# lim0606/pytorch-ardae-vae

Hardware: AMD Instinct MI355X
Metric: AR-DAE-VAE train-steps/sec (batch 512, nz_cdae 256) on dbMNIST (higher is better)
Workload: dtype f32; 1 GPU; BASELINE config #2: MNISTIPVAE mlp z=32 h=256 + cDAE mlp-grad h=256 L=3, global batch 512, nz_cdae 256 (131072 rows), dynamic binarisation on device, 1 cDAE + 1 VAE update per step; global_batch=512, nz_cdae=256, per_gpu_batch=512, parallelism=dp1

## Files before the change

### include/ardae_hip.h

```cpp
#ifndef ARDAE_HIP_H
#define ARDAE_HIP_H

#include <stddef.h>
#include <stdint.h>

#ifdef __cplusplus
extern "C" {
#endif

#define ARDAE_ABI_VERSION 1

enum { ARDAE_ACT_NONE = 0, ARDAE_ACT_RELU = 1, ARDAE_ACT_SOFTPLUS = 2, ARDAE_ACT_ELU = 3, ARDAE_ACT_TANH = 4, ARDAE_ACT_LEAKY_RELU = 5, ARDAE_ACT_SWISH = 6 };

enum {
  ARDAE_EPI_ACT = 0,
  ARDAE_EPI_DACT = 1,
  ARDAE_EPI_CHAIN = 2,
  ARDAE_EPI_DAE_LOSS = 3
};

typedef struct ardae_lin_src {
  const float* x;
  int ld;
  int K;
// ... 157 lines not shown
  int act;
  int flags;
} ardae_model_desc;
enum { ARDAE_MODEL_NO_CENTER = 1,
       ARDAE_MODEL_HEAD_SHIFT = 1, ARDAE_MODEL_HEAD_MASK = 7 << 1,
       ARDAE_MODEL_CLIPPED = 16,
       ARDAE_MODEL_CLIP_Z0_SHIFT = 8, ARDAE_MODEL_CLIP_Z_SHIFT = 12, ARDAE_MODEL_CLIP_MASK = 0xff00 };
size_t ardae_model_param_floats(const ardae_model_desc* d);
size_t ardae_model_packed_floats(const ardae_model_desc* d);
size_t ardae_model_workspace_floats(const ardae_model_desc* d, int B, int nz, int mode);
int ardae_model_pack(const ardae_model_desc* d, const float* params, float* packed, void* stream);
int ardae_model_encode(const ardae_model_desc* d, const float* params, const float* packed, const float* x,
                       const float* noise, int B, int nz, float* workspace, size_t workspace_floats, float* z_out,
                       void* stream);
int ardae_model_encode_pair(const ardae_model_desc* d, const float* params, const float* packed, const float* x,
                            const float* noise, int B, int nz, float* workspace, size_t workspace_floats, float* z0_out,
                            float* z_out, int phase, void* stream);
int ardae_model_vae_forward(const ardae_model_desc* d, const float* params, const float* packed, const float* x,
                            const float* noise, int B, int nz, float beta, float* workspace, size_t workspace_floats,
                            float* z_out, float* losses, void* stream);
int ardae_model_vae_forward_dev(const ardae_model_desc* d, const float* params, const float* packed, const float* x,
                                const float* noise, int B, int nz, const void* state, float* workspace, size_t workspace_floats,
                                float* z_out, float* losses, void* stream);
int ardae_model_encode_hidden(const ardae_model_desc* d, const float* params, const float* packed, const float* x, int B,
                              float* workspace, size_t workspace_floats, float* z0_out, float* hidden_out, void* stream);
int ardae_model_encode_hidden_raw(const ardae_model_desc* d, const float* params, const float* packed, const float* x, const float* raw0, int B,
                                  float* workspace, size_t workspace_floats, float* z0_out, float* hidden_out, void* stream);
int ardae_model_decode(const ardae_model_desc* d, const float* params, const float* packed, const float* z, int R,
                       float* workspace, size_t workspace_floats, float* out0, float* out1, void* stream);
int ardae_model_loss_rows(const ardae_model_desc* d, const float* out0, const float* out1, const float* x, const float* z,
                          int rows, int nz, float* recon_row, float* prior_row, void* stream);
int ardae_model_vae_backward(const ardae_model_desc* d, const float* params, const float* packed, const float* x,
                             const float* noise, int B, int nz, float beta, float dloss, const float* dz_extra,
                             float* workspace, size_t workspace_floats, float* grads, float grads_beta, void* stream);
int ardae_model_vae_backward_dev(const ardae_model_desc* d, const float* params, const float* packed, const float* x,
                                 const float* noise, int B, int nz, const void* state, float dloss, const float* dz_extra,
                                 float* workspace, size_t workspace_floats, float* grads, float grads_beta, void* stream);
int ardae_model_vae_backward_decoder(const ardae_model_desc* d, const float* params, const float* packed, const float* x,
                                     const float* noise, int B, int nz, float beta, float dloss, float* workspace,
                                     size_t workspace_floats, void* stream);
int ardae_model_vae_backward_sampler(const ardae_model_desc* d, const float* params, const float* packed, const float* x,
                                     const float* noise, int B, int nz, const float* dz_extra, float seed_scale,
                                     float* workspace, size_t workspace_floats, float* grads, float grads_beta, void* stream);
int ardae_model_vae_backward_decoder_dev(const ardae_model_desc* d, const float* params, const float* packed, const float* x,
                                         const float* noise, int B, int nz, const void* state, float dloss, float* workspace,
                                         size_t workspace_floats, void* stream);
// ... 93 lines not shown
```

### pytorch-ardae-vae_amd/csrc/host_util.h

```cpp
#pragma once
#include <algorithm>
#include <cstring>
#include <vector>

#include "common.h"
#include "elementwise.h"
#include "linear.h"
#include "wgrad.h"

namespace ardae {

inline size_t al64(size_t n) { return (n + 63) & ~size_t(63); }
inline unsigned nblk(int64_t n) { return (unsigned)((n + 255) / 256); }

struct Bump {
  float* base; size_t cap; size_t off = 0; bool ok = true;
  Bump(float* b, size_t c) : base(b), cap(c) {}
  Bump() : base(nullptr), cap(~size_t(0) >> 2) {}
  float* take(size_t n) {
    size_t o = off; off += al64(n);
    if (off > cap) { ok = false; return base; }
    return base ? base + o : nullptr;
  }
};

inline int lin1(int epi, int act, int M, int Nout, const float* x, int ldx, int K, const float* wp, LinArgs a, hipStream_t st) {
  a.M = M; a.Nout = Nout; a.nsrc = 1; a.act = act;
  a.src[0].x = x; a.src[0].ld = ldx; a.src[0].K = K; a.src[0].wp = wp;
  return launch_linear(a, epi, st);
}
inline int lin2(int epi, int act, int M, int Nout, const float* x0, int ld0, int K0, const float* wp0, const float* x1, int ld1, int K1, const float* wp1,
                LinArgs a, hipStream_t st) {
  a.M = M; a.Nout = Nout; a.nsrc = 2; a.act = act;
  a.src[0].x = x0; a.src[0].ld = ld0; a.src[0].K = K0; a.src[0].wp = wp0;
  a.src[1].x = x1; a.src[1].ld = ld1; a.src[1].K = K1; a.src[1].wp = wp1;
  return launch_linear(a, epi, st);
}

inline int dense_fwd(int act, int M, int n, const float* x, int ldx, int K, const float* wp, const float* bias, float* y, hipStream_t st) {
  LinArgs A{}; A.bias = bias; A.Y = y; A.ldY = n;
  return lin1(EPI_ACT, act, M, n, x, ldx, K, wp, A, st);
}
inline int dense_bwd(int act, int M, int n, const float* g, int K, const float* wp, const float* S, float* y, hipStream_t st, const float* Q = nullptr) {
  LinArgs A{}; A.S = S; A.ldS = n; A.Q = Q; A.ldQ = Q ? n : 0; A.Y = y; A.ldY = n;
  return lin1(EPI_DACT, act, M, n, g, K, K, wp, A, st);
}
inline int dense_bwd2(int act, int M, int n, const float* g0, const float* wp0, const float* g1, const float* wp1, int K, const float* S, float* y,
                      hipStream_t st) {
  LinArgs A{}; A.S = S; A.ldS = n; A.Y = y; A.ldY = n;
  return lin2(EPI_DACT, act, M, n, g0, K, K, wp0, g1, K, K, wp1, A, st);
}

struct Lin { size_t w, b; int out, in; };
inline Lin next_lin(size_t& off, int out, int in, int nbias = -1) {
  Lin l; l.out = out; l.in = in; l.w = off; off += (size_t)out * in; l.b = off; off += nbias < 0 ? out : nbias;
  return l;
}

struct PackList {
  std::vector<PackItem> items;
  const float* params; float* packed;
  size_t off = 0;
  PackList() : params(nullptr), packed(nullptr) {}
  PackList(const float* params_, float* packed_) : params(params_), packed(packed_) {}
// ... 82 lines not shown
       CAP_HIDDEN_RAW = 4 };
struct Family {
  int (*desc_check)(const ardae_model_desc* d);
  unsigned (*caps)(const ardae_model_desc& d);
  size_t (*param_floats)(const ardae_model_desc&);
  size_t (*packed_floats)(const ardae_model_desc&);
  size_t (*workspace_floats)(const ardae_model_desc&, int B, int nz, int mode);
  int (*pack)(const ardae_model_desc&, const float* params, float* packed, hipStream_t);
  int (*encode)(const ardae_model_desc&, const float* params, const float* packed, const float* x, const float* noise, int B, int nz,
                float* workspace, size_t wsf, float* z_out, float* hidden_out, hipStream_t, const float* raw0);
  int (*decode)(const ardae_model_desc&, const float* params, const float* packed, const float* z, int R, float* workspace, size_t wsf,
                float* out0, hipStream_t, float* out1);
  int (*vae_forward)(const ardae_model_desc&, const float* params, const float* packed, const float* x, const float* noise, int B, int nz,
                     DevFloat beta, float* workspace, size_t wsf, float* z_out, float* losses, hipStream_t);
  int (*vae_backward)(const ardae_model_desc&, const float* params, const float* packed, const float* x, const float* noise, int B, int nz,
                      DevFloat beta, float dloss, const float* dz_extra, float* workspace, size_t wsf, float* grads, float grads_beta, hipStream_t);
  const GaussFamily* gauss;
  int (*encode_pair)(const ardae_model_desc&, const float* params, const float* packed, const float* x, const float* noise, int B, int nz,
                     float* workspace, size_t wsf, float* z0_out, float* z_out, int phase, hipStream_t);
  int (*vae_backward_decoder)(const ardae_model_desc&, const float* params, const float* packed, const float* x, const float* noise, int B, int nz,
                              DevFloat beta, float dloss, float* workspace, size_t wsf, hipStream_t);
  int (*vae_backward_sampler)(const ardae_model_desc&, const float* params, const float* packed, const float* x, const float* noise, int B, int nz,
                              const float* dz_extra, DevFloat seed_scale, float* workspace, size_t wsf, float* grads, float grads_beta, hipStream_t);
};
inline unsigned no_caps(const ardae_model_desc&) { return 0; }
inline int desc_flags_ok(const ardae_model_desc* d, int allowed) {
  ARDAE_CHECK_ARG((d->flags & ~allowed) == 0,
                  "model: unknown flags %d (ARDAE_MODEL_NO_CENTER / the sampler-head bits / ARDAE_MODEL_CLIPPED: residual-conv kinds 5 / 6 only; "
                  "the log-variance clip codes: kinds 3 / 7 only)", d->flags);
  ARDAE_CHECK_ARG(((d->flags >> ARDAE_MODEL_CLIP_Z0_SHIFT) & 15) <= 10 && ((d->flags >> ARDAE_MODEL_CLIP_Z_SHIFT) & 15) <= 10, "model: unknown log-variance clip code");
  return 0;
}
const Family* family_of(int kind);
inline const Family& family(const ardae_model_desc* d) { return *family_of(d->kind); }

template <class Layout, class Packed> size_t family_param_floats(const ardae_model_desc& d) { return Layout(d).total; }
template <class Layout, class Packed> size_t family_packed_floats(const ardae_model_desc& d) {
  const Layout P(d);
  PackList pl;
  const Packed K(P, pl);
  return pl.total();
}
template <class Layout, class Packed> int family_pack(const ardae_model_desc& d, const float* params, float* packed, hipStream_t st) {
  const Layout P(d);
  PackList pl(params, packed);
  const Packed K(P, pl);
// ... 15 lines not shown
```

### pytorch-ardae-vae_amd/csrc/ipmodel.h

```cpp
#pragma once
#include "host_util.h"
#include "mlp.h"

namespace ardae {

struct IpBufs { float *z, *out0, *out1, *dout0, *dout1, *dzq, *dz, *rec_row, *pri_row; };

struct IpEncodeOut { float* z_out; float* hidden_out; const float* raw0; bool std0; };

struct IpTraitsBase {
  static constexpr bool mlp_decoder = false;
  static constexpr bool direct_z = false;
  struct Grads { float* grads; float beta; };
  template <class Entry> static Grads grads_of(Entry&, const float*, const float*, float* grads, float grads_beta) { return {grads, grads_beta}; }
  template <class Layout> static size_t extra_floats(const Layout&, int, int, int) { return 0; }
  template <class Layout> static int rows_ok(const Layout&, int, bool) { return 0; }
  template <class Entry> static int hidden_copy(Entry&, float*, int, hipStream_t) { return 0; }
};

template <class F> size_t ip_workspace_floats(const ardae_model_desc& d, int B, int nz, int mode) {
  const typename F::Layout P(d);
  const typename F::Packed K(P);
  if constexpr (F::mlp_decoder)
    if (mode == 2) return K.dec.decode_floats((size_t)B * nz);
  const int m = mode == 3 ? 0 : mode;
  Bump ws;
  typename F::Ws W{};
  carve(P, K, ws, B, nz, m, W);
  if (m == 1) {
    WgradList wl(nullptr);
    F::wgrads(P, K, W, nullptr, nullptr, B, nz, wl, ws);
  }
  return ws.off + F::extra_floats(P, B, nz, mode);
}

template <class F> int ip_encode(const ardae_model_desc& d, const float* params, const float* packed, const float* x, const float* noise, int B, int nz,
                                 float* workspace, size_t wsf, float* z_out, float* hidden_out, hipStream_t st, const float* raw0) {
  typename F::Entry entry(d, workspace, wsf, B, nz, 0);
  auto& [P, K, ws, W] = entry;
  const size_t nn = F::noise_floats(P, B, nz);
  float* zero = noise ? nullptr : F::zero_noise(entry, nn);
  ARDAE_CHECK_ARG(ws.ok, "model_encode: internal workspace accounting error");
  ARDAE_TRY(F::rows_ok(P, nz, true));
  ARDAE_CHECK_ARG(!hidden_out || nz == 1, "model_encode: the hidden context is defined for nz == 1");
  const IpEncodeOut enc{z_out, hidden_out, raw0, noise == nullptr};
  ARDAE_TRY(noise_or_zero(noise, zero, nn, st));
  ARDAE_TRY(F::sampler_fwd(entry, params, packed, x, noise, B, nz, &enc, st));
  if (z_out && !F::direct_z) ARDAE_TRY(launch_copy(F::bufs(W).z, (size_t)B * nz * d.z_dim, z_out, st));
  if (hidden_out) ARDAE_TRY(F::hidden_copy(entry, hidden_out, B, st));
  return 0;
}

template <class F> int ip_decode(const ardae_model_desc& d, const float* params, const float* packed, const float* z, int R, float* workspace, size_t wsf,
                                 float* out0, hipStream_t st, float*) {
  typename F::Entry entry(d, workspace, wsf, R, 1, 2);
  ARDAE_CHECK_ARG(entry.ws.ok, "model_decode: internal workspace accounting error");
  ARDAE_TRY(F::decoder_fwd(entry, params, packed, z, R, st));
  return launch_copy(F::bufs(entry.W).out0, (size_t)R * d.input_dim, out0, st);
}

template <class F> int ip_vae_forward(const ardae_model_desc& d, const float* params, const float* packed, const float* x, const float* noise, int B, int nz,
                                      DevFloat beta, float* workspace, size_t wsf, float* z_out, float* losses, hipStream_t st) {
  typename F::Entry entry(d, workspace, wsf, B, nz, 1);
  auto& [P, K, ws, W] = entry;
  ARDAE_CHECK_ARG(ws.ok, "model_vae_forward: internal workspace accounting error");
  ARDAE_TRY(F::rows_ok(P, nz, false));
  const IpBufs G = F::bufs(W);
  const int R = B * nz;
  ARDAE_TRY(F::sampler_fwd(entry, params, packed, x, noise, B, nz, nullptr, st));
  ARDAE_TRY(launch_copy(G.z, (size_t)R * d.z_dim, z_out, st));
  ARDAE_TRY(F::decoder_fwd(entry, params, packed, G.z, R, st));
  ARDAE_TRY(launch_vae_loss(G.out1 ? 1 : 0, G.out0, G.out1, x, G.z, R, nz, d.input_dim, d.z_dim, beta, 0, 0.f, nullptr, G.rec_row, G.pri_row, nullptr,
                            nullptr, nullptr, st));
  return launch_vae_loss_finalize(G.rec_row, G.pri_row, R, beta, losses, st);
}

template <class F> int ip_backward(const ardae_model_desc& d, const float* params, const float* packed, const float* x, const float* noise, int B, int nz,
                                   DevFloat beta, float dloss, const float* dz_extra, DevFloat seed_scale, float* workspace, size_t wsf, float* grads,
                                   float grads_beta, int phases, hipStream_t st) {
  typename F::Entry entry(d, workspace, wsf, B, nz, 1);
  ARDAE_CHECK_ARG(entry.ws.ok, "model_vae_backward: internal workspace accounting error");
  typename F::Grads g = F::grads_of(entry, params, packed, grads, grads_beta);
  const IpBufs G = F::bufs(entry.W);
  const int R = B * nz;
  if (phases & 1) {
    ARDAE_TRY(launch_vae_loss(G.out1 ? 1 : 0, G.out0, G.out1, x, G.z, R, nz, d.input_dim, d.z_dim, beta, 1, dloss / (float)R,
                              phases == 3 ? dz_extra : nullptr, G.rec_row, G.pri_row, G.dout0, G.dout1, G.dzq, st));
    ARDAE_TRY(F::decoder_bwd(entry, packed, R, g, st));
  }
  if (!(phases & 2)) return 0;
  if (phases == 2 && dz_extra) ARDAE_TRY(launch_axpy(dz_extra, (int64_t)R * d.z_dim, seed_scale, G.dz, st));
  return F::sampler_bwd(entry, params, packed, x, noise, B, nz, g, st);
}
template <class F> int ip_vae_backward(const ardae_model_desc& d, const float* params, const float* packed, const float* x, const float* noise, int B,
                                       int nz, DevFloat beta, float dloss, const float* dz_extra, float* workspace, size_t wsf, float* grads,
                                       float grads_beta, hipStream_t st) {
  return ip_backward<F>(d, params, packed, x, noise, B, nz, beta, dloss, dz_extra, 1.f, workspace, wsf, grads, grads_beta, 3, st);
// ... 25 lines not shown
```

### pytorch-ardae-vae_amd/csrc/mlp.h

```cpp
#pragma once
#include <vector>

#include "host_util.h"

namespace ardae {

struct MlpStack {
  std::vector<Lin> lin;
  std::vector<size_t> f, b;
  MlpStack() {}
  MlpStack(const Lin* l, size_t n, PackList& pl) : lin(l, l + n), f(n), b(n) {
    for (size_t i = 0; i < n; ++i) pl.pair(lin[i], f[i], b[i]);
  }
  size_t n() const { return lin.size(); }

  int fwd(const float* params, const float* packed, int act, int M, const float* x, float* const* a, hipStream_t st, size_t first = 1) const {
    for (size_t l = first; l <= n(); ++l) {
      const Lin& L = lin[l - 1];
      ARDAE_TRY(dense_fwd(act, M, L.out, l == 1 ? x : a[l - 1], L.in, L.in, packed + f[l - 1], params + L.b, a[l], st));
    }
    return 0;
  }
  int bwd(const float* packed, int act, int M, float* const* a, float* const* d, hipStream_t st) const {
    for (size_t l = n(); l >= 2; --l) ARDAE_TRY(dense_bwd(act, M, lin[l - 1].in, d[l], lin[l - 1].out, packed + b[l - 1], a[l - 1], d[l - 1], st));
    return 0;
  }
  void wgrads(WgradList& wl, int M, const float* x, float* const* a, float* const* d) const {
    for (size_t l = 1; l <= n(); ++l) {
      const Lin& L = lin[l - 1];
      wl.push(M, L.out, L.in, d[l], l == 1 ? x : a[l - 1], L.in, wl.g(L.w), L.in, wl.g(L.b));
    }
  }
  void carve(Bump& ws, size_t M, std::vector<float*>& a) const {
    a.assign(n() + 1, nullptr);
    for (size_t l = 1; l <= n(); ++l) a[l] = ws.take(M * lin[l - 1].out);
  }
};

struct MlpDecoder {
  MlpStack stack;
  Lin head[2];
  size_t head_f[2], head_b[2];
  int nh = 0;
// ... 73 lines not shown
```

### pytorch-ardae-vae_amd/csrc/model.hip

```cpp
#include <vector>

#include "ardae_hip.h"
#include "common.h"
#include "auxconvvae.h"
#include "auxmodel.h"
#include "auxvae.h"
#include "convmodel.h"
#include "convvae.h"
#include "resmodel.h"
#include "vaemodel.h"
#include "ipmodel.h"
#include "elementwise.h"
#include "mlp.h"

namespace ardae {
namespace {

struct ModelLayout {
  int kind, D, nd, h, zd, nl, act;
  std::vector<Lin> inp, stack, dec, heads;
  std::vector<bool> stack_noise;
  size_t total = 0;
  explicit ModelLayout(const ardae_model_desc& d)
      : kind(d.kind), D(d.input_dim), nd(d.noise_dim), h(d.h_dim), zd(d.z_dim), nl(d.n_layers), act(d.act) {
// ... 43 lines not shown
  float *rec_row, *pri_row;
  std::vector<float*> dt, de;
  float* drb;
};

void carve(const ModelLayout& P, const ModelPacked& K, Bump& ws, int B, int nz, int mode, ModelWs& W) {
  const size_t R = (size_t)B * nz, h = P.h;
  W.x2 = ws.take((size_t)B * P.D);
  K.inp.carve(ws, B, W.e);
  W.rb = ws.take((size_t)B * h);
  W.t.assign(P.stack.size(), nullptr);
  for (size_t i = 1; i < P.stack.size(); ++i) W.t[i] = ws.take(R * h);
  W.z = ws.take(R * P.zd);
  if (mode == 0) return;
  K.dec.carve(ws, R, true, W.D);
  W.rec_row = ws.take(R); W.pri_row = ws.take(R);
  W.dt.assign(P.stack.size(), nullptr);
  for (size_t i = 1; i < P.stack.size(); ++i) W.dt[i] = ws.take(R * h);
  K.inp.carve(ws, B, W.de);
  W.drb = ws.take((size_t)B * h);
}
using MlpEntry = Entry<ModelLayout, ModelPacked, ModelWs>;

int encode_trunk(const ModelLayout& P, const ModelPacked& K, const float* params, const float* packed, const float* x, int B,
                 ModelWs& W, hipStream_t st) {
  const int h = P.h;
  const float* x_in = x;
  if (P.kind == 0) {
    ARDAE_TRY(launch_affine(x, (int64_t)B * P.D, 2.f, -1.f, W.x2, st));
    x_in = W.x2;
  }
  ARDAE_TRY(K.inp.fwd(params, packed, P.act, B, x_in, W.e.data(), st));
  return dense_fwd(ACT_NONE, B, h, W.e[P.inp.size()], h, h, packed + K.sh_f[0], params + P.stack[0].b, W.rb, st);
}

int encode_stack(const ModelLayout& P, const ModelPacked& K, const float* params, const float* packed, const float* noise,
                 int B, int nz, const float* rb, const std::vector<float*>& t, float* zdst, bool keep_hidden, hipStream_t st) {
  const int R = B * nz, h = P.h, act = P.act;
  const size_t ns = P.stack.size();
  if (!keep_hidden && ns == 2 && P.stack_noise[0] && !P.stack_noise[1] && P.stack[0].out == h) {
    LinArgs A{}; A.M = R; A.Nout = h; A.act = act; A.nsrc = 1;
    A.rowbias = rb; A.rowbias_ld = h; A.rows_per_group = nz;
    A.src[0].x = noise; A.src[0].ld = P.nd; A.src[0].K = P.nd; A.src[0].wp = packed + K.sn_f[0];
    if (sampler_tail_eligible(A, P.stack[1].out))
      return launch_sampler_tail(A, packed + K.sh_f[1], params + P.stack[1].b, zdst, P.stack[1].out, P.stack[1].out, st);
  }
  for (size_t i = 0; i < ns; ++i) {
    const bool last = i + 1 == ns;
    const int out = P.stack[i].out;
    LinArgs A{}; A.Y = last ? zdst : t[i + 1]; A.ldY = out; A.M = R; A.Nout = out; A.act = last ? ACT_NONE : act;
    int n = 0;
    if (i == 0) {
      A.rowbias = rb; A.rowbias_ld = h; A.rows_per_group = nz;
    } else {
      A.bias = params + P.stack[i].b;
      A.src[n].x = t[i]; A.src[n].ld = h; A.src[n].K = h; A.src[n].wp = packed + K.sh_f[i]; ++n;
// ... 10 lines not shown
struct MlpTraits : IpTraitsBase {
  using Layout = ModelLayout; using Packed = ModelPacked; using Ws = ModelWs; using Entry = MlpEntry;
  static constexpr bool mlp_decoder = true;
  static constexpr bool direct_z = true;
  static int desc_check(const ardae_model_desc* d) { return mlp_desc_check(d, 0); }
  static unsigned caps(const ardae_model_desc& d) { return d.kind == 1 ? CAP_GAUSS_DECODER : 0; }
  static IpBufs bufs(const ModelWs& W) { return {W.z, W.D.o[0], W.D.o[1], W.D.dox[0], W.D.dox[1], W.D.dzq, W.D.dz, W.rec_row, W.pri_row}; }
  static void wgrads(const ModelLayout& P, const ModelPacked& K, const ModelWs& W, const float* x, const float* noise, int B, int nz, WgradList& wl, Bump& ws) {
    const int R = B * nz, h = P.h;
    const size_t ns = P.stack.size();
    K.dec.wgrads(wl, R, W.z, W.D);
    for (size_t i = 0; i < ns; ++i) {
      const Lin& L = P.stack[i];
      const float* G = (i == ns - 1) ? W.D.dz : W.dt[i + 1];
      if (i == 0) wl.push(B, L.out, h, W.drb, W.e[P.inp.size()], h, wl.g(L.w), L.in, nullptr);
      else wl.push(R, L.out, h, G, W.t[i], h, wl.g(L.w), L.in, P.stack_noise[i] ? nullptr : wl.g(L.b));
      if (P.stack_noise[i]) wl.push(R, L.out, P.nd, G, noise, P.nd, wl.g(L.w + h), L.in, wl.g(L.b));
    }
    K.inp.wgrads(wl, B, P.kind == 0 ? W.x2 : x, W.e.data(), W.de.data());
    wl.assign(ws, (int)(P.heads.size() + P.dec.size() + 2 * ns + P.inp.size()));
  }
  static size_t extra_floats(const ModelLayout& P, int B, int nz, int mode) {
    if (mode == 3) return (P.stack.size() - 1) * al64((size_t)B * P.h) + al64((size_t)B * P.nd);
    return al64((size_t)B * nz * P.nd);
  }
  static size_t noise_floats(const ModelLayout& P, int B, int nz) { return (size_t)B * nz * P.nd; }
  static float* zero_noise(Entry& e, size_t n) { return e.ws.take(n); }
  static int sampler_fwd(Entry& e, const float* params, const float* packed, const float* x, const float* noise, int B, int nz, const IpEncodeOut* enc,
                         hipStream_t st) {
    ARDAE_TRY(encode_trunk(e.P, e.K, params, packed, x, B, e.W, st));
    return encode_stack(e.P, e.K, params, packed, noise, B, nz, e.W.rb, e.W.t, enc && enc->z_out ? enc->z_out : e.W.z, enc == nullptr, st);
  }
  static int decoder_fwd(Entry& e, const float* params, const float* packed, const float* z, int R, hipStream_t st) {
    return e.K.dec.fwd(params, packed, e.P.act, R, z, e.W.D.hid.data(), e.W.D.o, st);
  }
  static int decoder_bwd(Entry& e, const float* packed, int R, Grads&, hipStream_t st) { return e.K.dec.bwd(packed, e.P.act, R, e.W.D, st); }
  static int sampler_bwd(Entry& e, const float*, const float* packed, const float* x, const float* noise, int B, int nz, Grads& g, hipStream_t st) {
    auto& [P, K, ws, W] = e;
    const int R = B * nz, h = P.h, act = P.act;
    const size_t ns = P.stack.size(), ninp = P.inp.size();
    for (size_t i = ns - 1; i >= 1; --i)
      ARDAE_TRY(dense_bwd(act, R, h, (i == ns - 1) ? W.D.dz : W.dt[i + 1], P.stack[i].out, packed + K.sh_b[i], W.t[i], W.dt[i], st));
    ARDAE_TRY(launch_segment_sum(W.dt[1], h, B, nz, h, 1.0f, W.drb, h, st));
    ARDAE_TRY(dense_bwd(act, B, h, W.drb, h, packed + K.sh_b[0], W.e[ninp], W.de[ninp], st));
    ARDAE_TRY(K.inp.bwd(packed, act, B, W.e.data(), W.de.data(), st));
    WgradList wl(g.grads, g.beta);
    wgrads(P, K, W, x, noise, B, nz, wl, ws);
    ARDAE_CHECK_ARG(ws.ok, "model_vae_backward: internal workspace accounting error");
    return wl.launch(st);
  }
};

int mlp_encode_pair(const ardae_model_desc& d, const float* params, const float* packed, const float* x, const float* noise, int B, int nz,
                    float* workspace, size_t wsf, float* z0_out, float* z_out, int phase, hipStream_t st) {
  MlpEntry entry(d, workspace, wsf, B, nz, 0);
  auto& [P, K, ws, W] = entry;
  std::vector<float*> t0(P.stack.size(), nullptr);
  for (size_t i = 1; i < P.stack.size(); ++i) t0[i] = ws.take((size_t)B * P.h);
  float* zero = ws.take((size_t)B * P.nd);
  ARDAE_CHECK_ARG(ws.ok, "model_encode_pair: internal workspace accounting error");
  if (phase != 2) {
    ARDAE_TRY(launch_fill(zero, (size_t)B * P.nd, 0.f, st));
    ARDAE_TRY(encode_trunk(P, K, params, packed, x, B, W, st));
    ARDAE_TRY(encode_stack(P, K, params, packed, zero, B, 1, W.rb, t0, z0_out, false, st));
  }
  if (phase != 1) ARDAE_TRY(encode_stack(P, K, params, packed, noise, B, nz, W.rb, W.t, z_out, false, st));
  return 0;
}

constexpr Family mlp_family() {
  Family f = ip_family<MlpTraits>();
  f.encode_pair = mlp_encode_pair;
  f.vae_backward_decoder = ip_vae_backward_decoder<MlpTraits>;
  f.vae_backward_sampler = ip_vae_backward_sampler<MlpTraits>;
  return f;
}
const Family MLP_FAMILY = mlp_family();

}

const Family* family_of(int kind) {
  static const Family* const by_kind[20] = {&MLP_FAMILY, &MLP_FAMILY, &CONV_FAMILY, &AUX_FAMILY, &AUXCONV_FAMILY, &RES_FAMILY, &RES_FAMILY, &AUX_FAMILY,
                                            &VAE_FAMILY, &VAE_FAMILY, nullptr, &CONVVAE_FAMILY, &RESVAE_FAMILY, nullptr, &AUXVAE_FAMILY,
                                            &AUXVAE_FAMILY, nullptr, &AUXCONVVAE_FAMILY, nullptr, &AUXRESVAE_FAMILY};
  return kind >= 0 && kind <= 19 ? by_kind[kind] : nullptr;
}

}

using namespace ardae;

static int desc_ok(const ardae_model_desc* d) {
  ARDAE_CHECK_ARG(d != nullptr, "model: desc is NULL");
  ARDAE_CHECK_ARG(family_of(d->kind) != nullptr,
                  "model: kind must be 0 (MNISTIPVAE), 1 (ToyIPVAE concat), 2 (ConvIPVAE), 3 (MNISTAuxIPVAE), 4 (MNISTConvAuxIPVAE), 5 (ResConvIPVAE), "
// ... 66 lines not shown
int ardae_model_decode(const ardae_model_desc* d, const float* params, const float* packed, const float* z, int R, float* workspace,
                       size_t workspace_floats_, float* out0, float* out1, void* stream) {
  ARDAE_TRY(desc_ok(d));
  ARDAE_CHECK_ARG(params && packed && z && workspace && out0 && R > 0, "model_decode: bad arguments");
  ARDAE_CHECK_ARG(!(family(d).caps(*d) & CAP_GAUSS_DECODER) || out1, "model_decode: the Gaussian decoder needs out1 (logvar)");
  ARDAE_CHECK_ARG(workspace_floats_ >= family(d).workspace_floats(*d, R, 1, 2), "model_decode: workspace too small");
  return family(d).decode(*d, params, packed, z, R, workspace, workspace_floats_, out0, (hipStream_t)stream, out1);
}

int ardae_model_loss_rows(const ardae_model_desc* d, const float* out0, const float* out1, const float* x, const float* z, int rows,
                          int nz, float* recon_row, float* prior_row, void* stream) {
  ARDAE_TRY(desc_ok(d));
  return launch_vae_loss(family(d).caps(*d) & CAP_GAUSS_DECODER ? 1 : 0, out0, out1, x, z, rows, nz, d->input_dim, d->z_dim, 1.f, 0, 0.f, nullptr, recon_row, prior_row, nullptr,
                         nullptr, nullptr, (hipStream_t)stream);
}

static int vae_forward_entry(const ardae_model_desc* d, const float* params, const float* packed, const float* x, const float* noise, int B,
                             int nz, DevFloat beta, float* workspace, size_t workspace_floats_, float* z_out, float* losses, void* stream) {
  ARDAE_TRY(model_common(d, params, packed, x, B, nz, workspace, workspace_floats_, 1));
  ARDAE_CHECK_ARG(noise && z_out && losses, "model_vae_forward: null pointer argument");
  return family(d).vae_forward(*d, params, packed, x, noise, B, nz, beta, workspace, workspace_floats_, z_out, losses, (hipStream_t)stream);
}

static int vae_backward_entry(const ardae_model_desc* d, const float* params, const float* packed, const float* x, const float* noise, int B,
                              int nz, DevFloat beta, float dloss, const float* dz_extra, float* workspace, size_t workspace_floats_,
                              float* grads, float grads_beta, void* stream) {
  ARDAE_TRY(model_common(d, params, packed, x, B, nz, workspace, workspace_floats_, 1));
  ARDAE_CHECK_ARG(noise && grads, "model_vae_backward: null pointer argument");
  return family(d).vae_backward(*d, params, packed, x, noise, B, nz, beta, dloss, dz_extra, workspace, workspace_floats_, grads, grads_beta,
                                (hipStream_t)stream);
}

static int vae_backward_decoder_entry(const ardae_model_desc* d, const float* params, const float* packed, const float* x, const float* noise,
                                      int B, int nz, DevFloat beta, float dloss, float* workspace, size_t workspace_floats_, void* stream) {
  ARDAE_TRY(model_common(d, params, packed, x, B, nz, workspace, workspace_floats_, 1));
  ARDAE_CHECK_ARG(noise, "model_vae_backward_decoder: null pointer argument");
  ARDAE_CHECK_ARG(family(d).vae_backward_decoder, "model_vae_backward_decoder: the conv model and the aux model have no split backward (use ardae_model_vae_backward)");
  return family(d).vae_backward_decoder(*d, params, packed, x, noise, B, nz, beta, dloss, workspace, workspace_floats_, (hipStream_t)stream);
}

static int vae_backward_sampler_entry(const ardae_model_desc* d, const float* params, const float* packed, const float* x, const float* noise,
                                      int B, int nz, const float* dz_extra, DevFloat seed_scale, float* workspace, size_t workspace_floats_,
                                      float* grads, float grads_beta, void* stream) {
  ARDAE_TRY(model_common(d, params, packed, x, B, nz, workspace, workspace_floats_, 1));
  ARDAE_CHECK_ARG(noise && grads, "model_vae_backward_sampler: null pointer argument");
  ARDAE_CHECK_ARG(family(d).vae_backward_sampler, "model_vae_backward_sampler: the conv model and the aux model have no split backward (use ardae_model_vae_backward)");
  return family(d).vae_backward_sampler(*d, params, packed, x, noise, B, nz, dz_extra, seed_scale, workspace, workspace_floats_, grads, grads_beta,
                                        (hipStream_t)stream);
}

int ardae_model_vae_forward(const ardae_model_desc* d, const float* params, const float* packed, const float* x, const float* noise,
                            int B, int nz, float beta, float* workspace, size_t workspace_floats_, float* z_out, float* losses,
                            void* stream) {
  return vae_forward_entry(d, params, packed, x, noise, B, nz, beta, workspace, workspace_floats_, z_out, losses, stream);
}
int ardae_model_vae_forward_dev(const ardae_model_desc* d, const float* params, const float* packed, const float* x, const float* noise,
                                int B, int nz, const void* state, float* workspace, size_t workspace_floats_, float* z_out, float* losses,
                                void* stream) {
  ARDAE_CHECK_ARG(state, "model_vae_forward_dev: state is NULL");
  return vae_forward_entry(d, params, packed, x, noise, B, nz, train_state_beta(state), workspace, workspace_floats_, z_out, losses, stream);
}

int ardae_model_vae_backward(const ardae_model_desc* d, const float* params, const float* packed, const float* x, const float* noise,
                             int B, int nz, float beta, float dloss, const float* dz_extra, float* workspace,
                             size_t workspace_floats_, float* grads, float grads_beta, void* stream) {
  return vae_backward_entry(d, params, packed, x, noise, B, nz, beta, dloss, dz_extra, workspace, workspace_floats_, grads, grads_beta, stream);
}
int ardae_model_vae_backward_dev(const ardae_model_desc* d, const float* params, const float* packed, const float* x, const float* noise,
                                 int B, int nz, const void* state, float dloss, const float* dz_extra, float* workspace,
                                 size_t workspace_floats_, float* grads, float grads_beta, void* stream) {
  ARDAE_CHECK_ARG(state, "model_vae_backward_dev: state is NULL");
  return vae_backward_entry(d, params, packed, x, noise, B, nz, train_state_beta(state), dloss, dz_extra, workspace, workspace_floats_, grads,
                            grads_beta, stream);
}

int ardae_model_vae_backward_decoder(const ardae_model_desc* d, const float* params, const float* packed, const float* x,
                                     const float* noise, int B, int nz, float beta, float dloss, float* workspace,
                                     size_t workspace_floats_, void* stream) {
  return vae_backward_decoder_entry(d, params, packed, x, noise, B, nz, beta, dloss, workspace, workspace_floats_, stream);
}
int ardae_model_vae_backward_decoder_dev(const ardae_model_desc* d, const float* params, const float* packed, const float* x,
                                         const float* noise, int B, int nz, const void* state, float dloss, float* workspace,
                                         size_t workspace_floats_, void* stream) {
  ARDAE_CHECK_ARG(state, "model_vae_backward_decoder_dev: state is NULL");
  return vae_backward_decoder_entry(d, params, packed, x, noise, B, nz, train_state_beta(state), dloss, workspace, workspace_floats_, stream);
// ... 18 lines not shown
```

### pytorch-ardae-vae_amd/engine.py

```python
import contextlib
from dataclasses import dataclass

import numpy as np
import torch

from . import _lib as L
from . import dist
from . import rng
from .iwae import IwaeEvaluator
from .diagnostics import PosteriorDiagnostics
from .engine_common import CaptureLadder, _FlatOpt, bump_versions, capture_linear, check_batch, check_tensor, rebuild_step_state
from .optim import WEIGHT_AVG_KINDS, unwrap_state_dict, wrap_state_dict


@dataclass
class TrainConfig:
    delta: float = 0.1
    std_scale: float = 1e4
    nz_cdae: int = 256
    nstd_cdae: int = 1
    nz_model: int = 1
    num_cdae_updates: int = 1
    beta: float = 1.0
    beta_init: float = None
# ... 62 lines not shown
        if self.comm is not None and (self.comm.world, self.comm.rank) != (self.world, self.rank):
            raise ValueError(f"dp_comm is rank {self.comm.rank} of {self.comm.world}, the process group says {self.rank} of {self.world}")
        md, cd = model._desc, cdae._desc
        B, nzc, nzm = self.B, cfg.nz_cdae, cfg.nz_model
        N = B * nzc
        z, nd = model.z_dim, model._noise_width
        if cfg.cdae_ctx_type not in ("lt0", "hidden1a", "data"):
            raise NotImplementedError(f"cdae_ctx_type {cfg.cdae_ctx_type!r}")
        if cfg.cdae_ctx_type == "hidden1a" and not model.hidden_dim:
            raise NotImplementedError("hidden1a is the aux models' context (ivae_ardae.py:572-580)")
        self.hidden_ctx = cfg.cdae_ctx_type == "hidden1a"
        self.data_ctx = cfg.cdae_ctx_type == "data"
        self.clipped = bool(getattr(model, "_clipped", False))
        if self.clipped and not self.hidden_ctx:
            raise NotImplementedError("MNISTResConvAuxIPVAEClipped is built with --cdae-ctx-type hidden1a (the aux models' context, ivae_ardae.py:572-580)")
        ctx_dim = model.hidden_dim if self.hidden_ctx else int(model.input_dim) if self.data_ctx else z
        if int(cdae.context_dim) != ctx_dim:
            raise ValueError(f"cdae.context_dim = {cdae.context_dim}, but the {cfg.cdae_ctx_type} context has {ctx_dim} columns")
        f = lambda *s: torch.empty(*s, device=self.dev, dtype=torch.float32)
        S = nzc * int(cfg.nstd_cdae)
        ws_floats = max(L.query("ardae_cdae_workspace_floats", cd, B, S, 1),
                        L.query("ardae_model_workspace_floats", md, B, nzc, 3))
        self.ws = f(ws_floats)
        self.ws_vae = f(L.query("ardae_model_workspace_floats", md, B, nzm, 1))
        self.ws_small = f(max(L.query("ardae_cdae_workspace_floats", cd, B, nzm, 0),
                              L.query("ardae_model_workspace_floats", md, B, 1, 0)))
        self.ws_small_v = f(L.query("ardae_model_workspace_floats", md, B, 1, 0))
        self.z0, self.latent = f(B, z), f(N, z)
        self.noise_s, self.xi, self.eps = f(model._noise_numel(B, nzc)), f(B * S), f(B * S, z)
        self.xbar, self.sigma, self.std_b = f(B * S, z), f(B * S), f(B)
        self.noise_v, self.zv, self.z0v, self.u, self.g = f(model._noise_numel(B, nzm)), f(B * nzm, z), f(B, z), f(B * nzm, z), f(B * nzm, z)
        self.sigma0 = torch.zeros(B * nzm, device=self.dev)
        if self.clipped:
            self.raw_c, self.raw_v = f(2, B, model.noise_dim), f(2, B, model.noise_dim)
        self.ctx_c, self.ctx_v = (f(B, ctx_dim), f(B, ctx_dim)) if (self.hidden_ctx or self.data_ctx) else (self.z0, self.z0v)
        if self.data_ctx:
            self._ctx_half = torch.full((B, ctx_dim), 0.5 if cfg.ctx_data_center else 0.0, device=self.dev)
        self.loss_c, self.losses_m = f(1), f(3)
        self.grads_c = torch.zeros_like(cdae._flat)
        self.grads_m = torch.zeros_like(model._flat)
        self.n_c = cdae._flat.numel() - (1 if cdae._kind == "grad" else 0)
        self.step_count = 0
        self.state = torch.zeros(4, dtype=torch.int64, device=self.dev)
        self.sched = cfg.beta_schedule()
        train = None if self.sched is None else self.sched + (float(cfg.std_scale), B * nzm)
        self.opt_m = _FlatOpt(cfg.m_optimizer, model._flat, model._flat.numel(), cfg.m_lr, cfg.m_beta1, cfg.d_momentum, state=self.state, train=train)
        self.opt_c = _FlatOpt(cfg.d_optimizer, cdae._flat, self.n_c, cfg.d_lr, cfg.d_beta1, cfg.d_momentum)
# ... 233 lines not shown
        L.call("ardae_cdae_loss_grads", self.cdae._desc, self.cdae._flat, self.pk_c, self.xbar, self.sigma, eps, self.ctx_c, B, nz * nstd,
               self.ws, self.ws.numel(), self.loss_c, self.grads_c, None)

    def _cdae_update(self):
        if self._in_step and self.opt_c.adam:
            self.opt_c.advance()
        self.opt_c.apply(self.grads_c, self._in_step)
        if not self._in_step:
            self.opt_c.steps += 1
        self._pack_cdae()

    def _data_context(self, x, out):
        D = int(self.model.input_dim)
        L.call("ardae_center_scale", x, self._ctx_half, self.B, 1, D, 2.0 if self.cfg.ctx_data_center else 1.0, out)

    def vae_forward_part(self, x, noise=None, beta=None, draw=None):
        self._require_trained("vae_forward_part()")
        self._check_batch(x, "vae_forward_part")
        cfg = self.cfg
        beta = self._beta_arg(beta)
        dev = "_dev" if beta is None else ""
        B, nz, md = self.B, cfg.nz_model, self.model._desc
        nv = noise["vae"] if noise else self._normal(self.noise_v, draw)
        L.call("ardae_model_vae_forward" + dev, md, self.model._flat, self.pk_m, x, nv, B, nz, self.state if dev else beta, self.ws_vae,
               self.ws_vae.numel(), self.zv, self.losses_m)
        if self.hidden_ctx:
            raws = None
            if self.clipped:
                if noise:
                    raws = torch.stack([noise["vctx_raw"].reshape(B, -1), noise["vz0_raw"].reshape(B, -1)]).float().contiguous()
                else:
                    raws = self._normal(self.raw_v, None if draw is None else 12)
            self._hidden(x, self.z0v, self.ctx_v, self.ws_small_v, raws)
        else:
            self._encode(x, None, 1, self.z0v, self.ws_small_v)
        if self.data_ctx:
            self._data_context(x, self.ctx_v)
        L.call("ardae_center_scale", self.zv, self.z0v, B, nz, self.model.z_dim, cfg.std_scale, self.u)
        if self.split_backward:
            L.call("ardae_model_vae_backward_decoder" + dev, md, self.model._flat, self.pk_m, x, nv, B, nz, self.state if dev else beta, 1.0,
                   self.ws_vae, self.ws_vae.numel())
        return nv

    def vae_backward_part(self, x, nv, beta=None, apply_update=True):
        self._require_trained("vae_backward_part()")
        self._vae_backward_grads(x, nv, beta)
        if self.dp:
            self._allreduce(self.grads_m)
        if apply_update:
# ... 446 lines not shown
```

Before: 217.2 train-steps/sec.

## Compute VAE forward and zero-noise encoding together sharing one encoder trunk

Adds a vae_forward_pair entry that runs the encoder trunk once. It then derives both the noisy-sample z and the deterministic z0, the zero-noise mean used for centring, from that shared trunk. Previously a separate encode pass recomputed the trunk. When the stack form allows, the zero-noise stack is folded into the trunk launch chain so no zero-noise buffer is filled, and the same path is used in encode_pair. This costs a larger workspace mode and more code paths with an eligibility check and a fallback.

```diff
diff --git a/include/ardae_hip.h b/include/ardae_hip.h
--- a/include/ardae_hip.h
+++ b/include/ardae_hip.h
@@ -203,6 +203,12 @@
 int ardae_model_vae_forward_dev(const ardae_model_desc* d, const float* params, const float* packed, const float* x,
                                 const float* noise, int B, int nz, const void* state, float* workspace, size_t workspace_floats,
                                 float* z_out, float* losses, void* stream);
+int ardae_model_vae_forward_pair(const ardae_model_desc* d, const float* params, const float* packed, const float* x,
+                                 const float* noise, int B, int nz, float beta, float* workspace, size_t workspace_floats,
+                                 float* z_out, float* z0_out, float* losses, void* stream);
+int ardae_model_vae_forward_pair_dev(const ardae_model_desc* d, const float* params, const float* packed, const float* x,
+                                     const float* noise, int B, int nz, const void* state, float* workspace, size_t workspace_floats,
+                                     float* z_out, float* z0_out, float* losses, void* stream);
 int ardae_model_encode_hidden(const ardae_model_desc* d, const float* params, const float* packed, const float* x, int B,
                               float* workspace, size_t workspace_floats, float* z0_out, float* hidden_out, void* stream);
 int ardae_model_encode_hidden_raw(const ardae_model_desc* d, const float* params, const float* packed, const float* x, const float* raw0, int B,
diff --git a/pytorch-ardae-vae_amd/csrc/host_util.h b/pytorch-ardae-vae_amd/csrc/host_util.h
--- a/pytorch-ardae-vae_amd/csrc/host_util.h
+++ b/pytorch-ardae-vae_amd/csrc/host_util.h
@@ -37,9 +37,14 @@
   return launch_linear(a, epi, st);
 }
 
+inline LinArgs dense_fwd_args(int act, int M, int n, const float* x, int ldx, int K, const float* wp, const float* bias, float* y) {
+  LinArgs A{}; A.bias = bias; A.Y = y; A.ldY = n;
+  A.M = M; A.Nout = n; A.nsrc = 1; A.act = act;
+  A.src[0].x = x; A.src[0].ld = ldx; A.src[0].K = K; A.src[0].wp = wp;
+  return A;
+}
 inline int dense_fwd(int act, int M, int n, const float* x, int ldx, int K, const float* wp, const float* bias, float* y, hipStream_t st) {
-  LinArgs A{}; A.bias = bias; A.Y = y; A.ldY = n;
-  return lin1(EPI_ACT, act, M, n, x, ldx, K, wp, A, st);
+  return launch_linear(dense_fwd_args(act, M, n, x, ldx, K, wp, bias, y), EPI_ACT, st);
 }
 inline int dense_bwd(int act, int M, int n, const float* g, int K, const float* wp, const float* S, float* y, hipStream_t st, const float* Q = nullptr) {
   LinArgs A{}; A.S = S; A.ldS = n; A.Q = Q; A.ldQ = Q ? n : 0; A.Y = y; A.ldY = n;
@@ -168,6 +173,8 @@
                               DevFloat beta, float dloss, float* workspace, size_t wsf, hipStream_t);
   int (*vae_backward_sampler)(const ardae_model_desc&, const float* params, const float* packed, const float* x, const float* noise, int B, int nz,
                               const float* dz_extra, DevFloat seed_scale, float* workspace, size_t wsf, float* grads, float grads_beta, hipStream_t);
+  int (*vae_forward_pair)(const ardae_model_desc&, const float* params, const float* packed, const float* x, const float* noise, int B, int nz,
+                          DevFloat beta, float* workspace, size_t wsf, float* z_out, float* z0_out, float* losses, hipStream_t);
 };
 inline unsigned no_caps(const ardae_model_desc&) { return 0; }
 inline int desc_flags_ok(const ardae_model_desc* d, int allowed) {
diff --git a/pytorch-ardae-vae_amd/csrc/ipmodel.h b/pytorch-ardae-vae_amd/csrc/ipmodel.h
--- a/pytorch-ardae-vae_amd/csrc/ipmodel.h
+++ b/pytorch-ardae-vae_amd/csrc/ipmodel.h
@@ -23,7 +23,7 @@
   const typename F::Packed K(P);
   if constexpr (F::mlp_decoder)
     if (mode == 2) return K.dec.decode_floats((size_t)B * nz);
-  const int m = mode == 3 ? 0 : mode;
+  const int m = mode == 3 ? 0 : mode == 5 ? 1 : mode;
   Bump ws;
   typename F::Ws W{};
   carve(P, K, ws, B, nz, m, W);
@@ -59,20 +59,23 @@
   return launch_copy(F::bufs(entry.W).out0, (size_t)R * d.input_dim, out0, st);
 }
 
-template <class F> int ip_vae_forward(const ardae_model_desc& d, const float* params, const float* packed, const float* x, const float* noise, int B, int nz,
-                                      DevFloat beta, float* workspace, size_t wsf, float* z_out, float* losses, hipStream_t st) {
-  typename F::Entry entry(d, workspace, wsf, B, nz, 1);
-  auto& [P, K, ws, W] = entry;
-  ARDAE_CHECK_ARG(ws.ok, "model_vae_forward: internal workspace accounting error");
-  ARDAE_TRY(F::rows_ok(P, nz, false));
-  const IpBufs G = F::bufs(W);
+template <class F> int ip_vae_forward_rest(typename F::Entry& entry, const ardae_model_desc& d, const float* params, const float* packed, const float* x, int B,
+                                           int nz, DevFloat beta, float* z_out, float* losses, hipStream_t st) {
+  const IpBufs G = F::bufs(entry.W);
   const int R = B * nz;
-  ARDAE_TRY(F::sampler_fwd(entry, params, packed, x, noise, B, nz, nullptr, st));
   ARDAE_TRY(launch_copy(G.z, (size_t)R * d.z_dim, z_out, st));
   ARDAE_TRY(F::decoder_fwd(entry, params, packed, G.z, R, st));
   ARDAE_TRY(launch_vae_loss(G.out1 ? 1 : 0, G.out0, G.out1, x, G.z, R, nz, d.input_dim, d.z_dim, beta, 0, 0.f, nullptr, G.rec_row, G.pri_row, nullptr,
                             nullptr, nullptr, st));
   return launch_vae_loss_finalize(G.rec_row, G.pri_row, R, beta, losses, st);
+}
+template <class F> int ip_vae_forward(const ardae_model_desc& d, const float* params, const float* packed, const float* x, const float* noise, int B, int nz,
+                                      DevFloat beta, float* workspace, size_t wsf, float* z_out, float* losses, hipStream_t st) {
+  typename F::Entry entry(d, workspace, wsf, B, nz, 1);
+  ARDAE_CHECK_ARG(entry.ws.ok, "model_vae_forward: internal workspace accounting error");
+  ARDAE_TRY(F::rows_ok(entry.P, nz, false));
+  ARDAE_TRY(F::sampler_fwd(entry, params, packed, x, noise, B, nz, nullptr, st));
+  return ip_vae_forward_rest<F>(entry, d, params, packed, x, B, nz, beta, z_out, losses, st);
 }
 
 template <class F> int ip_backward(const ardae_model_desc& d, const float* params, const float* packed, const float* x, const float* noise, int B, int nz,
diff --git a/pytorch-ardae-vae_amd/csrc/mlp.h b/pytorch-ardae-vae_amd/csrc/mlp.h
--- a/pytorch-ardae-vae_amd/csrc/mlp.h
+++ b/pytorch-ardae-vae_amd/csrc/mlp.h
@@ -14,11 +14,12 @@
   }
   size_t n() const { return lin.size(); }
 
+  LinArgs fwd_args(const float* params, const float* packed, int act, int M, const float* x, float* const* a, size_t l) const {
+    const Lin& L = lin[l - 1];
+    return dense_fwd_args(act, M, L.out, l == 1 ? x : a[l - 1], L.in, L.in, packed + f[l - 1], params + L.b, a[l]);
+  }
   int fwd(const float* params, const float* packed, int act, int M, const float* x, float* const* a, hipStream_t st, size_t first = 1) const {
-    for (size_t l = first; l <= n(); ++l) {
-      const Lin& L = lin[l - 1];
-      ARDAE_TRY(dense_fwd(act, M, L.out, l == 1 ? x : a[l - 1], L.in, L.in, packed + f[l - 1], params + L.b, a[l], st));
-    }
+    for (size_t l = first; l <= n(); ++l) ARDAE_TRY(launch_linear(fwd_args(params, packed, act, M, x, a, l), EPI_ACT, st));
     return 0;
   }
   int bwd(const float* packed, int act, int M, float* const* a, float* const* d, hipStream_t st) const {
diff --git a/pytorch-ardae-vae_amd/csrc/model.hip b/pytorch-ardae-vae_amd/csrc/model.hip
--- a/pytorch-ardae-vae_amd/csrc/model.hip
+++ b/pytorch-ardae-vae_amd/csrc/model.hip
@@ -89,16 +89,47 @@
 }
 using MlpEntry = Entry<ModelLayout, ModelPacked, ModelWs>;
 
+struct Std0Out { const std::vector<float*>* t0; float* z0; };
+
+void trunk_links(const ModelLayout& P, const ModelPacked& K, const float* params, const float* packed, const float* x_in, int B, ModelWs& W,
+                 const Std0Out* std0, std::vector<LinArgs>& ch) {
+  const int h = P.h, n = (int)P.inp.size();
+  for (int l = 1; l <= n; ++l) ch.push_back(K.inp.fwd_args(params, packed, P.act, B, x_in, W.e.data(), l));
+  ch.push_back(dense_fwd_args(ACT_NONE, B, h, W.e[n], h, h, packed + K.sh_f[0], params + P.stack[0].b, W.rb));
+  if (!std0) return;
+  const std::vector<float*>& t0 = *std0->t0;
+  const size_t ns = P.stack.size();
+  ch.push_back(dense_fwd_args(P.act, B, h, W.e[n], h, h, packed + K.sh_f[0], params + P.stack[0].b, t0[1]));
+  for (size_t i = 1; i < ns; ++i) {
+    const bool last = i + 1 == ns;
+    ch.push_back(dense_fwd_args(last ? ACT_NONE : P.act, B, P.stack[i].out, t0[i], h, h, packed + K.sh_f[i], params + P.stack[i].b, last ? std0->z0 : t0[i + 1]));
+  }
+}
+bool std0_form_ok(const ModelLayout& P, const ModelPacked& K, const float* packed, int B, const float* zero) {
+  if (P.stack[0].out != P.h) return false;
+  LinArgs A = dense_fwd_args(P.act, B, P.h, zero, P.nd, P.nd, packed + K.sn_f[0], nullptr, nullptr);
+  A.Y = const_cast<float*>(zero);
+  if (!linear_small_eligible(A, EPI_ACT)) return false;
+  A.Nout = P.stack.back().out;
+  if (!linear_small_eligible(A, EPI_ACT)) return false;
+  A.Nout = P.h; A.Y = nullptr; A.rowbias = zero; A.rowbias_ld = P.h; A.rows_per_group = 1;
+  return !sampler_tail_eligible(A, P.stack.back().out);
+}
+
+int trunk_input(const ModelLayout& P, const float* x, int B, ModelWs& W, const float*& x_in, hipStream_t st) {
+  x_in = x;
+  if (P.kind != 0) return 0;
+  x_in = W.x2;
+  return launch_affine(x, (int64_t)B * P.D, 2.f, -1.f, W.x2, st);
+}
 int encode_trunk(const ModelLayout& P, const ModelPacked& K, const float* params, const float* packed, const float* x, int B,
-                 ModelWs& W, hipStream_t st) {
-  const int h = P.h;
-  const float* x_in = x;
-  if (P.kind == 0) {
-    ARDAE_TRY(launch_affine(x, (int64_t)B * P.D, 2.f, -1.f, W.x2, st));
-    x_in = W.x2;
-  }
-  ARDAE_TRY(K.inp.fwd(params, packed, P.act, B, x_in, W.e.data(), st));
-  return dense_fwd(ACT_NONE, B, h, W.e[P.inp.size()], h, h, packed + K.sh_f[0], params + P.stack[0].b, W.rb, st);
+                 ModelWs& W, hipStream_t st, const Std0Out* std0 = nullptr) {
+  const float* x_in;
+  ARDAE_TRY(trunk_input(P, x, B, W, x_in, st));
+  std::vector<LinArgs> ch;
+  trunk_links(P, K, params, packed, x_in, B, W, std0, ch);
+  for (const LinArgs& a : ch) ARDAE_TRY(launch_linear(a, EPI_ACT, st));
+  return 0;
 }
 
 int encode_stack(const ModelLayout& P, const ModelPacked& K, const float* params, const float* packed, const float* noise,
@@ -155,6 +186,12 @@
   }
   static size_t extra_floats(const ModelLayout& P, int B, int nz, int mode) {
     if (mode == 3) return (P.stack.size() - 1) * al64((size_t)B * P.h) + al64((size_t)B * P.nd);
+    if (mode == 5) {
+      Bump ws;
+      ModelWs W;
+      carve(P, ModelPacked(P), ws, B, 1, 0, W);
+      return ws.off + extra_floats(P, B, 1, 0);
+    }
     return al64((size_t)B * nz * P.nd);
   }
   static size_t noise_floats(const ModelLayout& P, int B, int nz) { return (size_t)B * nz * P.nd; }
@@ -192,7 +229,10 @@
   for (size_t i = 1; i < P.stack.size(); ++i) t0[i] = ws.take((size_t)B * P.h);
   float* zero = ws.take((size_t)B * P.nd);
   ARDAE_CHECK_ARG(ws.ok, "model_encode_pair: internal workspace accounting error");
-  if (phase != 2) {
+  if (phase != 2 && std0_form_ok(P, K, packed, B, zero)) {
+    const Std0Out std0{&t0, z0_out};
+    ARDAE_TRY(encode_trunk(P, K, params, packed, x, B, W, st, &std0));
+  } else if (phase != 2) {
     ARDAE_TRY(launch_fill(zero, (size_t)B * P.nd, 0.f, st));
     ARDAE_TRY(encode_trunk(P, K, params, packed, x, B, W, st));
     ARDAE_TRY(encode_stack(P, K, params, packed, zero, B, 1, W.rb, t0, z0_out, false, st));
@@ -201,9 +241,33 @@
   return 0;
 }
 
+int mlp_vae_forward_pair(const ardae_model_desc& d, const float* params, const float* packed, const float* x, const float* noise, int B, int nz,
+                         DevFloat beta, float* workspace, size_t wsf, float* z_out, float* z0_out, float* losses, hipStream_t st) {
+  MlpEntry entry(d, workspace, wsf, B, nz, 1);
+  auto& [P, K, ws, W] = entry;
+  {
+    WgradList wl(nullptr);
+    MlpTraits::wgrads(P, K, W, nullptr, nullptr, B, nz, wl, ws);
+  }
+  const size_t tailf = MlpTraits::extra_floats(P, B, nz, 5);
+  float* tail = ws.take(tailf);
+  ARDAE_CHECK_ARG(ws.ok, "model_vae_forward_pair: internal workspace accounting error");
+  Bump tw(tail, tailf);
+  std::vector<float*> t0(P.stack.size(), nullptr);
+  for (size_t i = 1; i < P.stack.size(); ++i) t0[i] = tw.take((size_t)B * P.h);
+  const bool form = tw.ok && std0_form_ok(P, K, packed, B, tail);
+  const Std0Out std0{&t0, z0_out};
+  ARDAE_TRY(encode_trunk(P, K, params, packed, x, B, W, st, form ? &std0 : nullptr));
+  ARDAE_TRY(encode_stack(P, K, params, packed, noise, B, nz, W.rb, W.t, W.z, true, st));
+  ARDAE_TRY(ip_vae_forward_rest<MlpTraits>(entry, d, params, packed, x, B, nz, beta, z_out, losses, st));
+  if (form) return 0;
+  return ip_encode<MlpTraits>(d, params, packed, x, nullptr, B, 1, tail, tailf, z0_out, nullptr, st, nullptr);
+}
+
 constexpr Family mlp_family() {
   Family f = ip_family<MlpTraits>();
   f.encode_pair = mlp_encode_pair;
+  f.vae_forward_pair = mlp_vae_forward_pair;
   f.vae_backward_decoder = ip_vae_backward_decoder<MlpTraits>;
   f.vae_backward_sampler = ip_vae_backward_sampler<MlpTraits>;
   return f;
@@ -316,6 +380,17 @@
   return family(d).vae_forward(*d, params, packed, x, noise, B, nz, beta, workspace, workspace_floats_, z_out, losses, (hipStream_t)stream);
 }
 
+static int vae_forward_pair_entry(const ardae_model_desc* d, const float* params, const float* packed, const float* x, const float* noise, int B,
+                                  int nz, DevFloat beta, float* workspace, size_t workspace_floats_, float* z_out, float* z0_out, float* losses,
+                                  void* stream) {
+  ARDAE_TRY(desc_ok(d));
+  ARDAE_CHECK_ARG(family(d).vae_forward_pair, "model_vae_forward_pair: the MLP samplers only (kinds 0 / 1): use ardae_model_vae_forward and ardae_model_encode");
+  ARDAE_TRY(model_common(d, params, packed, x, B, nz, workspace, workspace_floats_, 5));
+  ARDAE_CHECK_ARG(noise && z_out && z0_out && losses, "model_vae_forward_pair: null pointer argument");
+  return family(d).vae_forward_pair(*d, params, packed, x, noise, B, nz, beta, workspace, workspace_floats_, z_out, z0_out, losses,
+                                    (hipStream_t)stream);
+}
+
 static int vae_backward_entry(const ardae_model_desc* d, const float* params, const float* packed, const float* x, const float* noise, int B,
                               int nz, DevFloat beta, float dloss, const float* dz_extra, float* workspace, size_t workspace_floats_,
                               float* grads, float grads_beta, void* stream) {
@@ -355,6 +430,19 @@
   return vae_forward_entry(d, params, packed, x, noise, B, nz, train_state_beta(state), workspace, workspace_floats_, z_out, losses, stream);
 }
 
+int ardae_model_vae_forward_pair(const ardae_model_desc* d, const float* params, const float* packed, const float* x, const float* noise,
+                                 int B, int nz, float beta, float* workspace, size_t workspace_floats_, float* z_out, float* z0_out,
+                                 float* losses, void* stream) {
+  return vae_forward_pair_entry(d, params, packed, x, noise, B, nz, beta, workspace, workspace_floats_, z_out, z0_out, losses, stream);
+}
+int ardae_model_vae_forward_pair_dev(const ardae_model_desc* d, const float* params, const float* packed, const float* x, const float* noise,
+                                     int B, int nz, const void* state, float* workspace, size_t workspace_floats_, float* z_out,
+                                     float* z0_out, float* losses, void* stream) {
+  ARDAE_CHECK_ARG(state, "model_vae_forward_pair_dev: state is NULL");
+  return vae_forward_pair_entry(d, params, packed, x, noise, B, nz, train_state_beta(state), workspace, workspace_floats_, z_out, z0_out, losses,
+                                stream);
+}
+
 int ardae_model_vae_backward(const ardae_model_desc* d, const float* params, const float* packed, const float* x, const float* noise,
                              int B, int nz, float beta, float dloss, const float* dz_extra, float* workspace,
                              size_t workspace_floats_, float* grads, float grads_beta, void* stream) {
diff --git a/pytorch-ardae-vae_amd/engine.py b/pytorch-ardae-vae_amd/engine.py
--- a/pytorch-ardae-vae_amd/engine.py
+++ b/pytorch-ardae-vae_amd/engine.py
@@ -108,7 +108,8 @@
         ws_floats = max(L.query("ardae_cdae_workspace_floats", cd, B, S, 1),
                         L.query("ardae_model_workspace_floats", md, B, nzc, 3))
         self.ws = f(ws_floats)
-        self.ws_vae = f(L.query("ardae_model_workspace_floats", md, B, nzm, 1))
+        self.forward_pair = not self.hidden_ctx and int(md.kind) < 2 and L.debug_knob("ARDAE_VAE_FORWARD_PAIR", "1") != "0"
+        self.ws_vae = f(L.query("ardae_model_workspace_floats", md, B, nzm, 5 if self.forward_pair else 1))
         self.ws_small = f(max(L.query("ardae_cdae_workspace_floats", cd, B, nzm, 0),
                               L.query("ardae_model_workspace_floats", md, B, 1, 0)))
         self.ws_small_v = f(L.query("ardae_model_workspace_floats", md, B, 1, 0))
@@ -388,9 +389,15 @@
         dev = "_dev" if beta is None else ""
         B, nz, md = self.B, cfg.nz_model, self.model._desc
         nv = noise["vae"] if noise else self._normal(self.noise_v, draw)
-        L.call("ardae_model_vae_forward" + dev, md, self.model._flat, self.pk_m, x, nv, B, nz, self.state if dev else beta, self.ws_vae,
-               self.ws_vae.numel(), self.zv, self.losses_m)
-        if self.hidden_ctx:
+        if self.forward_pair:
+            L.call("ardae_model_vae_forward_pair" + dev, md, self.model._flat, self.pk_m, x, nv, B, nz, self.state if dev else beta, self.ws_vae,
+                   self.ws_vae.numel(), self.zv, self.z0v, self.losses_m)
+        else:
+            L.call("ardae_model_vae_forward" + dev, md, self.model._flat, self.pk_m, x, nv, B, nz, self.state if dev else beta, self.ws_vae,
+                   self.ws_vae.numel(), self.zv, self.losses_m)
+        if self.forward_pair:
+            pass
+        elif self.hidden_ctx:
             raws = None
             if self.clipped:
                 if noise:
```

Result: no change. 217.6 train-steps/sec, median of 5 (+0.2%).
